# Shashank8834/multimodal-fl-security

Hardware: AMD Instinct MI355X
Metric: FL rounds/sec + aggregate-ms, K=128 clients 10M-param multimodal, 1/2/4/8 GPU (higher is better)
Workload: dtype f32 (bf16x6-split MFMA conv/GEMM = fp32 operands; Krum Gram bf16x4 hi/lo split, fp32 accumulate); 1 GPU; C3: Multi-Krum K=128, 20% sign-flip, ResNet-18 img + 1-layer GRU text late fusion, 5 local SGD steps/round; Krum distances reference-exact; preset=C3, model=resnet18-img+gru1-text late-fusion, clients=128, params=11800394, local_steps=5, batch=32, defense=krum(f=25, multi_k=64), attack=sign_flip, attackers=25, client_chunk=128, exchange=alltoall, krum_distances=reference-exact (fp32 torch.norm accumulation, D bit-identical to krum.py:89-97), training_phase=one captured HIP graph per round; local updates = one flr_train_clients_ex call

## Files before the change

### include/flr.h

```cpp
#ifndef FLR_H
#define FLR_H

#include <stddef.h>
#include <stdint.h>

#ifdef __cplusplus
extern "C" {
#endif

#define FLR_OK 0
#define FLR_ERR_ARG (-1)
#define FLR_ERR_HIP (-2)
#define FLR_ERR_UNSUPPORTED (-3)
#define FLR_ERR_WORKSPACE (-4)
#define FLR_ERR_KRUM_N (-5)

const char* flr_version(void);
const char* flr_build_info(void);
int flr_set_knob(const char* name, const char* value);
const char* flr_status_string(int status);
const char* flr_last_error(void);

size_t flr_pairwise_l2_workspace(int64_t K, int64_t P);
int flr_pairwise_l2(const float* X, int64_t K, int64_t P, int64_t ldx,
// ... 249 lines not shown
                          void* workspace, size_t workspace_bytes, void* stream);
int flr_conv2d_bwd_data_t_add(const float* dy, const float* w_t, const float* add,
                              float* dx, int64_t K, int64_t B, int64_t Cin, int64_t H,
                              int64_t W, int64_t Cout, int64_t KH, int64_t KW,
                              int64_t stride, int64_t pad, void* workspace,
                              size_t workspace_bytes, void* stream);
int flr_conv2d_fwd_t_ex(const float* x, const float* w_t, int64_t w_stride, float* y,
                        int64_t K, int64_t B, int64_t Cin, int64_t H, int64_t W, int64_t Cout,
                        int64_t KH, int64_t KW, int64_t stride, int64_t pad, void* workspace,
                        size_t workspace_bytes, void* stream);
int flr_conv2d_bwd_data_t_ex(const float* dy, const float* w_t, int64_t w_stride,
                             const float* add, float* dx, int64_t K, int64_t B, int64_t Cin,
                             int64_t H, int64_t W, int64_t Cout, int64_t KH, int64_t KW,
                             int64_t stride, int64_t pad, void* workspace,
                             size_t workspace_bytes, void* stream);
int flr_conv2d_resident_ok(int64_t K, int64_t B, int64_t Cin, int64_t H, int64_t W,
                           int64_t Cout, int64_t KH, int64_t KW, int64_t stride,
                           int64_t pad, int dgrad);
int flr_conv2d_bwd_weight_t(const float* x, const float* dy, float* dw_t, int64_t K,
                            int64_t B, int64_t Cin, int64_t H, int64_t W,
                            int64_t Cout, int64_t KH, int64_t KW, int64_t stride,
                            int64_t pad, int zero_dead_taps, void* workspace,
                            size_t workspace_bytes, void* stream);
int64_t flr_conv2d_bwd_weight_t_sq_slots(int64_t K, int64_t B, int64_t Cin, int64_t H,
                                         int64_t W, int64_t Cout, int64_t KH, int64_t KW,
                                         int64_t stride, int64_t pad);
int flr_conv2d_bwd_weight_t_sq(const float* x, const float* dy, float* dw_t, int64_t K,
                               int64_t B, int64_t Cin, int64_t H, int64_t W,
                               int64_t Cout, int64_t KH, int64_t KW, int64_t stride,
                               int64_t pad, int zero_dead_taps, double* sq, int64_t sq_ld,
// ... 190 lines not shown
```

### multimodal-fl-security_amd/csrc/conv_t_kernels.h

```cpp
#pragma once

#include "conv_t_plans.h"

namespace flr {
namespace convt {

__device__ __forceinline__ void xcd_tile(int& bx, int& by, int& bz) {
  const int gx = (int)gridDim.x, gy = (int)gridDim.y;
  const int n = gx * gy * (int)gridDim.z;
  const int lid = (int)blockIdx.x + gx * ((int)blockIdx.y + gy * (int)blockIdx.z);
  const int xcd = lid & 7, slot = lid >> 3;
  const int q = n >> 3, r = n & 7;
  const int t = (xcd < r ? xcd * (q + 1) : r * (q + 1) + (xcd - r) * q) + slot;
  bx = t % gx;
  by = (t / gx) % gy;
  bz = t / (gx * gy);
}

template <class P> struct has_sq : std::false_type {};
template <bool V> struct has_sq<WgtT<V>> : std::true_type {};

__device__ __forceinline__ double block_sumsq(double s, double* red) {
#pragma unroll
  for (int o = 32; o > 0; o >>= 1) s += __shfl_xor(s, o, 64);
// ... 307 lines not shown
  }
}

constexpr int SB = 32;
constexpr int TERM_B = 64 * SB;
__device__ __forceinline__ int zimg(int row, int c) {
  const int f = ((row >> 2) & 1) | ((((row >> 1) ^ (row >> 3)) & 1) << 1);
  return row * SB + 8 * (c ^ f);
}
constexpr int SG_OCC = 2;
template <class P> struct has_k8 : std::false_type {};
template <> struct has_k8<FwdT> : std::true_type {};
template <> struct has_k8<DgradT> : std::true_type {};
template <int A, int B> struct has_k8<BGemm<A, B>> : std::true_type {};
template <class Plan, int MS, int NS, int ABL = 0, bool NAR = false>
__device__ __forceinline__ void sgemm_body(const Plan& pl, int S, float* __restrict__ part, int remap) {
  static_assert(!NAR || (NS == 1 && (MS == 2 || MS == 4)), "narrow tiles: 128 or 256 x 32");
  constexpr int MSW = NAR ? MS / 2 : MS;
  __shared__ __attribute__((aligned(16))) __bf16 Ls[MS + NS][3][TERM_B];
  int bx = (int)blockIdx.x, by = (int)blockIdx.y, bz = (int)blockIdx.z;
  if (remap & 1) xcd_tile(bx, by, bz);
  if (remap >> 8) odd_slot_controls(remap);
  const int k = bz / S, split = bz % S;
  const int M = pl.M(), N = pl.N(), R = pl.R();
  const int ktiles = cdiv(R, BK);
  const int rbeg = (int)((int64_t)ktiles * split / S) * BK;
  const int rend = std::min(R, (int)((int64_t)ktiles * (split + 1) / S) * BK);
  const int m0 = by * BM * MS, n0 = bx * BN * NS;
  const int tid = threadIdx.x;
  const int wave = tid >> 6, lane = tid & 63;
  const int wm = wave >> 1, wn = wave & 1;
  const int h = lane >> 5, l32 = lane & 31;
  const int srowA = stash_row<Plan::QUAD_A>(tid), skA = stash_k<Plan::QUAD_A>(tid);
  const int srowB = stash_row<Plan::QUAD_B>(tid), skB = stash_k<Plan::QUAD_B>(tid);

  typename Plan::State8 sa[MS], sb[NS];
#pragma unroll
  for (int i = 0; i < MS; ++i) sa[i] = pl.init8(k, m0 + BM * i, n0, tid);
#pragma unroll
  for (int j = 0; j < NS; ++j) sb[j] = pl.init8(k, m0, n0 + BN * j, tid);
  float ra[MS][8], rb[NS][8];
  bf16x8 pa[MS][3], pb[NS][3];
  f32x16 acc[MSW][NS];
#pragma unroll
  for (int i = 0; i < MSW; ++i)
#pragma unroll
    for (int j = 0; j < NS; ++j)
#pragma unroll
      for (int e = 0; e < 16; ++e) acc[i][j][e] = 0.f;
  auto a_sub = [&](int i) { return NAR ? (wave * MSW + i) >> 1 : i; };
  auto a_row = [&](int i) { return NAR ? 32 * ((wave * MSW + i) & 1) + l32 : 32 * wm + l32; };
  auto b_row = [&]() { return NAR ? l32 : 32 * wn + l32; };
  auto m_off = [&](int i) { return NAR ? 32 * (wave * MSW + i) : BM * i + 32 * wm; };
  auto n_off = [&](int j) { return NAR ? 0 : BN * j + 32 * wn; };
  auto load = [&](int r) {
#pragma unroll
    for (int i = 0; i < MS; ++i) pl.load_a8(sa[i], r, ra[i]);
#pragma unroll
    for (int j = 0; j < NS; ++j) pl.load_b8(sb[j], r, rb[j]);
  };
  auto split_all = [&]() {
#pragma unroll
    for (int i = 0; i < MS; ++i) split3(ra[i], pa[i][0], pa[i][1], pa[i][2]);
#pragma unroll
    for (int j = 0; j < NS; ++j) split3(rb[j], pb[j][0], pb[j][1], pb[j][2]);
  };
  auto write_all = [&]() {
#pragma unroll
    for (int i = 0; i < MS; ++i)
// ... 38 lines not shown
    split_all();
    write_all();
    load(std::min(rbeg + BK, rlast));
    __syncthreads();
    auto tile_body = [&](int t) {
      const int r0 = rbeg + t * BK;
      if constexpr (!(ABL & 16)) compute_tile();
      if constexpr (!(ABL & 8)) split_all();
      if constexpr (!(ABL & 4)) __syncthreads();
      if constexpr (!(ABL & 2)) write_all();
      if constexpr (!(ABL & 1)) load(std::min(r0 + 2 * BK, rlast));
      __syncthreads();
    };
    for (int t = 0; t < ntile; ++t) tile_body(t);
  }
  TileOffs<MSW, NS> off;
#pragma unroll
  for (int i = 0; i < MSW; ++i) off.m[i] = m_off(i);
#pragma unroll
  for (int j = 0; j < NS; ++j) off.n[j] = n_off(j);
  off.wr = off.wc = 0;
  store_tiles<Plan, MSW, NS>(pl, S, part, k, split, m0, n0, h, l32, M, N, acc, off);
}

template <class Plan, int MS, int NS, int ABL = 0, bool NAR = false>
__global__ __launch_bounds__(THREADS, SG_OCC) void sgemm_kernel(const Plan pl, int S, float* __restrict__ part,
                                                                 int remap) {
  sgemm_body<Plan, MS, NS, ABL, NAR>(pl, S, part, remap);
}

constexpr int RES_N = 128;
constexpr int RES_IMG = (RES_N + 1) * SB;

template <class Plan>
__global__ __launch_bounds__(THREADS, SG_OCC) void rgemm_kernel(const Plan pl, int remap) {
  __shared__ __attribute__((aligned(16))) __bf16 La[3][TERM_B];
  __shared__ __attribute__((aligned(16))) __bf16 Lb[2][3][RES_IMG];
// ... 511 lines not shown
  return v ? v : conv_min_kt();
}

inline int dgrad_min_kt2() {
  static const int v = [] {
    const char* e = flr::knob("FLR_DGRAD_MINKT2");
    const int x = e ? atoi(e) : 0;
    return x >= 1 && x <= 256 ? x : 8;
  }();
  return v;
}

template <class Plan>
inline int plan_min_kt(const Plan& pl) {
  if (std::is_base_of<BGemmArgs, Plan>::value) return bgemm_min_kt();
  if constexpr (std::is_same<Plan, DgradT>::value) return pl.g.stride == 1 ? dgrad_min_kt1() : dgrad_min_kt2();
  return conv_min_kt();
}

template <class Plan>
size_t splits_bytes(const Plan& pl) {
  int S = 1;
  for (int sub : {1, 2, 3, 4}) S = std::max(S, choose_splits(pl.M(), pl.N(), pl.R(), pl.g.Kc, sub, plan_min_kt(pl)));
  return S > 1 ? (size_t)S * pl.g.Kc * pl.M() * pl.N() * sizeof(float) : 0;
}

inline int tile_choice(int M, int N, int R) {
  const char* e = flr::knob("FLR_CONV_TILE");
  const int forced = e ? atoi(e) : 0;
  if (forced == 11) return 11;
  if (forced == 21 && M % 128 == 0) return 21;
// ... 267 lines not shown
      case 13: return launch_tiles<Plan, 1, 3>(pl, ws, ws_bytes, st, name);
      case 31: return launch_tiles<Plan, 3, 1>(pl, ws, ws_bytes, st, name);
      case 14: return launch_tiles<Plan, 1, 4>(pl, ws, ws_bytes, st, name);
      case 41: return launch_tiles<Plan, 4, 1>(pl, ws, ws_bytes, st, name);
      default: break;
    }
  }
  switch (tile) {
    case 21: return launch_tiles<Plan, 2, 1>(pl, ws, ws_bytes, st, name);
    case 12: return launch_tiles<Plan, 1, 2>(pl, ws, ws_bytes, st, name);
    case 22: return launch_tiles<Plan, 2, 2>(pl, ws, ws_bytes, st, name);
    default: return launch_tiles<Plan, 1, 1>(pl, ws, ws_bytes, st, name);
  }
}

inline bool shape_ok(int64_t Cin, int64_t Cout) { return Cin % 64 == 0 && Cout % 64 == 0; }

inline bool args_ok(int64_t K, int64_t B, int64_t Cin, int64_t H, int64_t W, int64_t Cout, int64_t KH, int64_t KW,
                    int64_t stride, int64_t pad) {
  if (!conv::geom_ok(K, B, Cin, H, W, Cout, KH, KW, stride, pad) || !shape_ok(Cin, Cout)) return false;
  if (!(B * K * Cin * H * W * 4 < (int64_t(1) << 31) && B * K * Cout * H * W * 4 < (int64_t(1) << 31) &&
        KH * KW * Cin * Cout * 4 < (int64_t(1) << 31)))
    return false;
  if (stride > 4) return false;
  const conv::Geom g = conv::make_geom(K, B, Cin, H, W, Cout, KH, KW, stride, pad);
  if (!g.rect.ok) return false;
  DgradT cls[MAX_CLASSES];
  const int nc = dgrad_classes(g, cls);
  for (int c = 0; c < nc; ++c)
    if (!cls[c].crect.ok) return false;
// ... 6 lines not shown
```

### multimodal-fl-security_amd/csrc/conv_t_plans.h

```cpp
#pragma once

#include "conv_t_prims.h"

namespace flr {
namespace convt {

struct FwdT {
  static constexpr bool QUAD_A = false, QUAD_B = false;
  Geom g;
  const float* x;
  const float* w;
  float* y;
  int64_t wsk;
  static constexpr int LA = KR_VEC, LB = KR_GATHER;
  __host__ __device__ __forceinline__ int M() const { return g.Cout; }
  __host__ __device__ __forceinline__ int N() const { return g.B * g.Ho * g.Wo; }
  __host__ __device__ __forceinline__ int R() const { return g.ntaps * g.Cin; }
  struct State {
    rsrc_t ra, rb;
    unsigned a0;
    int ih0, iw0, xoff;
    bool nok;
  };
  __device__ __forceinline__ State init(int k, int m0, int n0, int tid) const {
// ... 103 lines not shown
  __device__ __forceinline__ void res_shift(int slot, int& dh, int& dw) const {
    int kh, kw;
    slot_tap(g, slot, kh, kw);
    dh = kh - g.pad;
    dw = kw - g.pad;
  }
};

struct DgradT {
  static constexpr bool QUAD_A = true, QUAD_B = false;
  Geom g;
  const float* dy;
  const float* w;
  float* dx;
  const float* add;
  int64_t wsk;
  int ca, cb, Hc, Wc, ntc;
  conv::FastDiv d_hcwc, d_wc;
  int8_t ckh[conv::MAXTAPS], ckw[conv::MAXTAPS];
  conv::TapRect crect;
  static constexpr int LA = RK_VEC, LB = KR_GATHER;
  __host__ __device__ __forceinline__ int M() const { return g.Cin; }
  __host__ __device__ __forceinline__ int N() const { return g.B * Hc * Wc; }
  __host__ __device__ __forceinline__ int R() const { return ntc * g.Cout; }
  struct State {
    rsrc_t ra, rb;
    unsigned a0;
    int ih, iw, yoff;
    bool nok;
  };
// ... 35 lines not shown
    const int nh = s.ih - kh, nw = s.iw - kw;
    const int oh = g.stride == 1 ? nh : nh / g.stride, ow = g.stride == 1 ? nw : nw / g.stride;
    const bool ok = s.nok & (nh >= 0) & (nw >= 0) & (oh < g.Ho) & (ow < g.Wo);
    const unsigned addr = (unsigned)((s.yoff + oh * g.Wo + ow) * 4);
    const unsigned vb = ok ? addr : SENT;
    const int cs = (int)g.syc;
    const int cb0 = co0 * cs * 4;
#pragma unroll
    for (int i = 0; i < 8; ++i) b[i] = ld1(s.rb, vb, cb0 + i * 4 * cs * 4);
  }
  __device__ __forceinline__ void store(int k, int m, int n, float v) const {
    const uint32_t bb = udiv(n, d_hcwc), p = n - bb * Hc * Wc;
    const uint32_t ihc = udiv(p, d_wc), iwc = p - ihc * Wc;
    const int ih = ca + (int)ihc * g.stride, iw = cb + (int)iwc * g.stride;
    const int64_t i = k * g.sxk + m * g.sxc + bb * g.sxb + ih * g.W + iw;
    dx[i] = add ? __fadd_rn(v, add[i]) : v;
  }
  __device__ __forceinline__ int64_t index(int k, int m, int n) const {
    const uint32_t bb = udiv(n, d_hcwc), p = n - bb * Hc * Wc;
    const uint32_t ihc = udiv(p, d_wc), iwc = p - ihc * Wc;
    const int ih = ca + (int)ihc * g.stride, iw = cb + (int)iwc * g.stride;
    return k * g.sxk + m * g.sxc + bb * g.sxb + ih * g.W + iw;
  }
  __device__ __forceinline__ bool linear() const { return g.stride == 1; }
  __device__ __forceinline__ float* out() const { return dx; }
  __device__ __forceinline__ int64_t tile_base(int k, int m0, int n0) const { return k * g.sxk + m0 * g.sxc + n0; }
  __device__ __forceinline__ int64_t ldm() const { return g.sxc; }
  struct State8 {
    rsrc_t ra, rb;
    unsigned a0;
    int ih, iw, yoff;
    bool nok;
// ... 54 lines not shown
  }
  __device__ __forceinline__ void res_shift(int slot, int& dh, int& dw) const {
    int kh, kw;
    conv::rect_tap(crect, slot, kh, kw);
    dh = g.pad - kh;
    dw = g.pad - kw;
  }
};

inline int dgrad_classes(const Geom& g, DgradT* out) {
  int n = 0;
  for (int ca = 0; ca < std::min(g.stride, g.H); ++ca)
    for (int cb = 0; cb < std::min(g.stride, g.W); ++cb) {
      DgradT& c = out[n++];
      c.g = g;
      c.ca = ca;
      c.cb = cb;
      c.Hc = (g.H - ca + g.stride - 1) / g.stride;
      c.Wc = (g.W - cb + g.stride - 1) / g.stride;
      c.d_hcwc = conv::make_fastdiv((uint32_t)(c.Hc * c.Wc));
      c.d_wc = conv::make_fastdiv((uint32_t)c.Wc);
      c.ntc = 0;
      for (int t = 0; t < g.ntaps; ++t) {
        const int kh = g.tap_kh[t], kw = g.tap_kw[t];
        if (((ca + g.pad - kh) % g.stride + g.stride) % g.stride != 0) continue;
        if (((cb + g.pad - kw) % g.stride + g.stride) % g.stride != 0) continue;
        c.ckh[c.ntc] = (int8_t)kh;
        c.ckw[c.ntc] = (int8_t)kw;
        ++c.ntc;
      }
// ... 661 lines not shown
```

### multimodal-fl-security_amd/csrc/train_clients.hip

```cpp
#include "flr_common.h"
#include "side_stream.h"

#include <algorithm>
#include <cstring>
#include <string>
#include <vector>

namespace flr {
int clip_sumsq_blocks(const float* const* g_blocks, const int64_t* numel, const int64_t* client_stride,
                      int64_t nblocks, int64_t K, double* out, int64_t out_ld, int nslots, hipStream_t st);
namespace tc {

constexpr int THREADS = 256;

__global__ void permute_images_kernel(const float* __restrict__ src, float* __restrict__ dst, int64_t K, int64_t B,
                                      int64_t C, int64_t HW) {
  const int64_t n = K * B * C * HW;
  for (int64_t i = (int64_t)blockIdx.x * THREADS + threadIdx.x; i < n; i += (int64_t)gridDim.x * THREADS) {
    const int64_t p = i % HW, r = i / HW;
    const int64_t b = r % B, r2 = r / B;
    const int64_t c = r2 % C, k = r2 / C;
    dst[i] = src[((k * B + b) * C + c) * HW + p];
  }
}
// ... 415 lines not shown
      t.n[i] = r[i].second;
      total = std::max(total, r[i].second);
    }
    const int64_t g = std::max<int64_t>(1, std::min<int64_t>(256, (total / 4 + THREADS - 1) / THREADS));
    hipLaunchKernelGGL(dead_ranges_kernel, dim3((unsigned)g, (unsigned)K_), dim3(THREADS), 0, st, t, gtrain, X, ld,
                       (int)std::min<int64_t>(nneg, K_));
    return launch_status("train_clients: dead ranges");
  }

  struct Options {
    AuxStream* side = nullptr;
    AuxStream* text = nullptr;
    AuxStream* wgrad = nullptr;
    float* norms = nullptr;
    bool fuse_res = true;
    bool shared_first = true;
    float* xout = nullptr;
    int64_t xld = 0, xneg = 0;
  };
  void configure(const Options& o) { o_ = o; }

  int step(const float* images, const int64_t* tokens, const int64_t* labels, const float* mask, bool first,
           bool last, float* loss_row, float lr, float mom, hipStream_t st) {
    int rc;
    const int64_t C0 = s_.in_channels, HW0 = s_.image_size * s_.image_size;
    const Param& whh = ps_[p_whh_];
    Step S;
    S.st = st;
    S.conc = o_.text != nullptr;
    S.ts = S.conc ? o_.text->s : st;
// ... 218 lines not shown
    return FLR_OK;
  }

  int trunk_backward(Step& S) {
    int rc;
    const hipStream_t st = S.st;
    const int wg_text = S.conc ? [] {
      const char* e = flr::knob("FLR_WG_TEXT");
      return e ? atoi(e) : 2;
    }() : 0;
    for (int bi = (int)blocks_.size() - 1; bi >= 0; --bi) {
      Block& bk = blocks_[bi];
      S.wg_on_text = bi < wg_text;
      const float* d_out = bi + 1 < (int)blocks_.size() ? blocks_[bi + 1].d_in : d_x4_;
      FLR_TRY(bn_bwd(bk.b2, d_out, bk.y2, bk.out, true, bk.d_y2, bk.d_res, st));
      FLR_TRY(conv_bwd(S, bk.c2, bk.a1, bk.d_y2, bk.d_a1, st));
      FLR_TRY(bn_bwd(bk.b1, bk.d_a1, bk.y1, bk.a1, true, bk.d_y1, nullptr, st));
      const float* other = bk.d_res;
      if (bk.has_ds) {
        FLR_TRY(bn_bwd(bk.bds, bk.d_res, bk.yd, nullptr, false, bk.d_yd, nullptr, st));
        if (ps_[bk.c1.p].tap && ps_[bk.ds.p].tap && o_.fuse_res) {
          FLR_TRY(conv_bwd(S, bk.c1, bk.x_in, bk.d_y1, bk.d_in, st));
          FLR_TRY(conv_bwd(S, bk.ds, bk.x_in, bk.d_yd, bk.d_in, st, bk.d_in));
          continue;
        }
        FLR_TRY(conv_bwd(S, bk.ds, bk.x_in, bk.d_yd, bk.d_xd, st));
        other = bk.d_xd;
      }
      if (ps_[bk.c1.p].tap && o_.fuse_res) {
        FLR_TRY(conv_bwd(S, bk.c1, bk.x_in, bk.d_y1, bk.d_in, st, other));
      } else {
        FLR_TRY(conv_bwd(S, bk.c1, bk.x_in, bk.d_y1, bk.d_xm, st));
// ... 171 lines not shown
  const float* tap_w(const Param& p, bool shared, int64_t& stride) const {
    stride = shared ? 0 : p.n;
    return shared ? gshared_ + p.off : p.w;
  }
  int conv_fwd(const Step& S, const ConvOp& c, const float* x, float* y, hipStream_t st, char* wsp = nullptr) {
    const Param& p = ps_[c.p];
    if (p.tap) {
      int64_t wst;
      const float* w = tap_w(p, S.wsh, wst);
      return flr_conv2d_fwd_t_ex(x, w, wst, y, K_, B_, c.Cin, c.H, c.H, c.Cout, c.k, c.k, c.stride, c.pad,
                                 wsp ? wsp : cws_, cws_n_, st);
    }
    return flr_conv2d_fwd(x, p.w, y, K_, B_, c.Cin, c.H, c.H, c.Cout, c.k, c.k, c.stride, c.pad, c.fws, c.fws_n, st);
  }
  int conv_bwd(Step& S, const ConvOp& c, const float* x, const float* dy, float* dx, hipStream_t st,
               const float* add = nullptr) {
    const Param& p = ps_[c.p];
    int rc;
    if (p.tap) {
      int64_t wst;
      const float* w = tap_w(p, S.wsh, wst);
      hipStream_t ws = st;
      char* wsp = cws_;
      if (S.wg_on_text && S.tx.left(2)) {
        FLR_TRY(ev_link(S.tx.take(), st, o_.text->s, "train_clients: text-stream weight-gradient fork"));
        ws = o_.text->s;
        wsp = cws3_;
      } else if (S.wg.left(2)) {
        FLR_TRY(ev_link(S.wg.take(), st, o_.wgrad->s, "train_clients: weight-gradient fork"));
        ws = o_.wgrad->s;
        wsp = cws2_;
      }
      if (dx && (rc = flr_conv2d_bwd_data_t_ex(dy, w, wst, add, dx, K_, B_, c.Cin, c.H, c.H, c.Cout, c.k, c.k,
                                               c.stride, c.pad, cws_, cws_n_, st)) != FLR_OK)
        return rc;
      const int zero_dead = p.dead ? 0 : 1;
      if (p.sq_base >= 0)
        return flr_conv2d_bwd_weight_t_sq(x, dy, p.g, K_, B_, c.Cin, c.H, c.H, c.Cout, c.k, c.k, c.stride, c.pad,
                                          zero_dead, sq_ + p.sq_base, std::max<int64_t>(1, nsq_), wsp, cws_n_, ws);
      return flr_conv2d_bwd_weight_t(x, dy, p.g, K_, B_, c.Cin, c.H, c.H, c.Cout, c.k, c.k, c.stride, c.pad, zero_dead,
                                     wsp, cws_n_, ws);
    }
    if (dx && (rc = flr_conv2d_bwd_data(dy, p.w, dx, K_, B_, c.Cin, c.H, c.H, c.Cout, c.k, c.k, c.stride, c.pad, cws_,
                                        cws_n_, st)) != FLR_OK)
      return rc;
    return flr_conv2d_bwd_weight_reuse(x, dy, p.g, K_, B_, c.Cin, c.H, c.H, c.Cout, c.k, c.k, c.stride, c.pad, c.fws,
                                       c.fws_n, st);
  }
  int bn_fwd(const BnOp& b, const float* x, const float* res, float* y, bool relu, hipStream_t st) {
    return flr_batchnorm_fwd(x, ps_[b.pg].w, ps_[b.pb].w, res, y, b.mean, b.invstd, 1, K_ * b.C, b.HW, 1e-5f,
                             relu ? 1 : 0, st);
  }
  int bn_bwd(const BnOp& b, const float* dy, const float* x, const float* y, bool relu, float* dx, float* dres,
             hipStream_t st) {
    return flr_batchnorm_bwd(dy, x, relu ? y : nullptr, ps_[b.pg].w, b.mean, b.invstd, dx, ps_[b.pg].g, ps_[b.pb].g,
                             dres, 1, K_ * b.C, b.HW, relu ? 1 : 0, st);
  }
  int gemm(const float* A, int64_t ak, int64_t am, int64_t ar, const float* Bm, int64_t bk, int64_t bn, int64_t br,
           float* C, int64_t ck, int64_t cm, int64_t cn, const float* bias, int64_t bias_k, const float* add,
           int64_t M, int64_t N, int64_t R, hipStream_t st) {
    return flr_bgemm(A, ak, am, ar, Bm, bk, bn, br, C, ck, cm, cn, bias, bias_k, add, K_, M, N, R, gws_, gws_n_, st);
  }
// ... 89 lines not shown
  float* step_loss = reinterpret_cast<float*>(base + align_up(net.bytes(), 256));
  static const bool fuse_res = [] {
    const char* e = flr::knob("FLR_FUSED_RES");
    return !(e && e[0] == '0');
  }();
  static const bool shared_first = [] {
    const char* e = flr::knob("FLR_SHARED_FIRST");
    return !(e && e[0] == '0');
  }();
  const bool train_order = (flags & FLR_TC_TRAIN_ORDER) != 0;
  hipStream_t st = as_stream(stream);
  tc::Net::Options o;
  o.norms = norms_out;
  o.fuse_res = fuse_res;
  o.shared_first = shared_first;
  o.side = side_stream(true, st);
  o.text = text_stream(true, st);
  o.wgrad = wgrad_stream(true, st);
  if (train_order) {
    o.xout = X;
    o.xld = ld;
    o.xneg = nneg;
  }
  net.configure(o);
  rc = train_order ? net.load_global_train(global, st) : net.load_global(global, st);
  if (rc != FLR_OK) return rc;
  const int64_t C0 = spec->in_channels, HW0 = spec->image_size * spec->image_size, T = spec->seq_len;
  for (int64_t s = 0; s < steps; ++s) {
    rc = net.step(images + s * K * B * C0 * HW0, tokens + s * K * B * T, labels + s * K * B,
                  dropout_masks ? dropout_masks + s * K * B * spec->fusion : nullptr, s == 0, s == steps - 1,
// ... 51 lines not shown
```

### multimodal-fl-security_amd/csrc/train_conv_t_dgrad.hip

```cpp
#include "conv_t_kernels.h"

using namespace flr;

extern "C" int flr_conv2d_bwd_data_t(const float* dy, const float* w_t, float* dx, int64_t K, int64_t B, int64_t Cin,
                                     int64_t H, int64_t W, int64_t Cout, int64_t KH, int64_t KW, int64_t stride,
                                     int64_t pad, void* ws, size_t ws_bytes, void* stream) {
  return flr_conv2d_bwd_data_t_add(dy, w_t, nullptr, dx, K, B, Cin, H, W, Cout, KH, KW, stride, pad, ws, ws_bytes,
                                   stream);
}

extern "C" int flr_conv2d_bwd_data_t_add(const float* dy, const float* w_t, const float* add, float* dx, int64_t K,
                                         int64_t B, int64_t Cin, int64_t H, int64_t W, int64_t Cout, int64_t KH,
                                         int64_t KW, int64_t stride, int64_t pad, void* ws, size_t ws_bytes,
                                         void* stream) {
  return flr_conv2d_bwd_data_t_ex(dy, w_t, KH * KW * Cin * Cout, add, dx, K, B, Cin, H, W, Cout, KH, KW, stride, pad,
                                  ws, ws_bytes, stream);
}

extern "C" int flr_conv2d_bwd_data_t_ex(const float* dy, const float* w_t, int64_t w_stride, const float* add,
                                        float* dx, int64_t K, int64_t B, int64_t Cin, int64_t H, int64_t W,
                                        int64_t Cout, int64_t KH, int64_t KW, int64_t stride, int64_t pad, void* ws,
                                        size_t ws_bytes, void* stream) {
  if (!dy || !w_t || !dx || w_stride < 0) return FLR_ERR_ARG;
  if (!convt::args_ok(K, B, Cin, H, W, Cout, KH, KW, stride, pad))
    return conv::geom_ok(K, B, Cin, H, W, Cout, KH, KW, stride, pad) ? FLR_ERR_UNSUPPORTED : FLR_ERR_ARG;
  if (stride > 4) return FLR_ERR_UNSUPPORTED;
  const conv::Geom g = conv::make_geom(K, B, Cin, H, W, Cout, KH, KW, stride, pad);
  convt::DgradT cls[convt::MAX_CLASSES];
  const int nc = convt::dgrad_classes(g, cls);
  for (int c = 0; c < nc; ++c) {
    if (add == dx && cls[c].R() == 0) continue;
    cls[c].dy = dy; cls[c].w = w_t; cls[c].dx = dx; cls[c].add = add; cls[c].wsk = w_stride;
    const int rc = convt::launch(cls[c], ws, ws_bytes, as_stream(stream), "conv bwd data (tap-major)");
    if (rc != FLR_OK) return rc;
  }
  return FLR_OK;
}
```

### multimodal-fl-security_amd/flr/_capi.py

```python
from __future__ import annotations

import ctypes
import os
import threading

import torch

_PKG_ROOT = os.path.dirname(os.path.dirname(os.path.abspath(__file__)))
LIB_PATH = os.environ.get("FLR_LIB", os.path.join(_PKG_ROOT, "lib", "libflr.so"))
HEADER_PATH = os.path.join(os.path.dirname(_PKG_ROOT), "include", "flr.h")

FLR_OK = 0
FLR_ERR_ARG = -1
FLR_ERR_HIP = -2
FLR_ERR_UNSUPPORTED = -3
FLR_ERR_WORKSPACE = -4
FLR_ERR_KRUM_N = -5

_c_void_p = ctypes.c_void_p
_i64 = ctypes.c_int64
_size_t = ctypes.c_size_t
_int = ctypes.c_int

SIGNATURES = {
# ... 116 lines not shown
    "flr_vit_bert_num_params": (_i64, [_c_void_p]),
    "flr_train_vit_bert_workspace": (_size_t, [_c_void_p, _i64, _i64, _i64, _i64]),
    "flr_train_vit_bert": (_int, [_c_void_p, _c_void_p, _c_void_p, _i64, _c_void_p, _c_void_p, _c_void_p,
                                  _c_void_p, _i64, _i64, _i64, ctypes.c_float, ctypes.c_float, ctypes.c_float,
                                  ctypes.c_float, _i64, _c_void_p, _c_void_p, ctypes.c_uint, _i64, _c_void_p,
                                  _size_t, _c_void_p]),
    "flr_conv2d_tap_major_ok": (_int, [_i64, _i64]),
    "flr_conv2d_t_workspace": (_size_t, [_i64] * 10),
    "flr_conv2d_fwd_t": (_int, [_c_void_p, _c_void_p, _c_void_p] + [_i64] * 10 + [_c_void_p, _size_t, _c_void_p]),
    "flr_conv2d_bwd_data_t": (_int, [_c_void_p, _c_void_p, _c_void_p] + [_i64] * 10 + [_c_void_p, _size_t, _c_void_p]),
    "flr_conv2d_bwd_data_t_add": (_int, [_c_void_p] * 4 + [_i64] * 10 + [_c_void_p, _size_t, _c_void_p]),
    "flr_conv2d_fwd_t_ex": (_int, [_c_void_p, _c_void_p, _i64, _c_void_p] + [_i64] * 10 + [_c_void_p, _size_t,
                                                                                          _c_void_p]),
    "flr_conv2d_bwd_data_t_ex": (_int, [_c_void_p, _c_void_p, _i64, _c_void_p, _c_void_p] + [_i64] * 10 +
                                 [_c_void_p, _size_t, _c_void_p]),
    "flr_conv2d_resident_ok": (_int, [_i64] * 10 + [_int]),
    "flr_conv2d_bwd_weight_t": (_int, [_c_void_p, _c_void_p, _c_void_p] + [_i64] * 10 + [_int, _c_void_p, _size_t,
                                                                                         _c_void_p]),
    "flr_conv2d_bwd_weight_t_sq_slots": (_i64, [_i64] * 10),
    "flr_conv2d_wgrad_resident_ok": (_int, [_i64] * 10),
    "flr_conv2d_bwd_weight_t_sq": (_int, [_c_void_p, _c_void_p, _c_void_p] + [_i64] * 10 + [_int, _c_void_p, _i64,
                                                                                            _c_void_p, _size_t,
                                                                                            _c_void_p]),
    "flr_conv2d_fwd": (_int, [_c_void_p, _c_void_p, _c_void_p] + [_i64] * 10 + [_c_void_p, _size_t, _c_void_p]),
    "flr_conv2d_bwd_data": (_int, [_c_void_p, _c_void_p, _c_void_p] + [_i64] * 10 + [_c_void_p, _size_t, _c_void_p]),
    "flr_conv2d_bwd_weight": (_int, [_c_void_p, _c_void_p, _c_void_p] + [_i64] * 10 + [_c_void_p, _size_t, _c_void_p]),
    "flr_conv2d_bwd_weight_reuse": (_int, [_c_void_p, _c_void_p, _c_void_p] + [_i64] * 10 + [_c_void_p, _size_t,
                                                                                            _c_void_p]),
    "flr_cross_entropy": (_int, [_c_void_p, _c_void_p, _i64, _i64, _i64, _c_void_p, _c_void_p, _c_void_p, _c_void_p]),
    "flr_mean_rows": (_int, [_c_void_p, _i64, _i64, _c_void_p, _c_void_p]),
# ... 132 lines not shown
```

Before: 17.65 rounds/s.

## Merge strided dgrad phase classes into one launch and fold shortcut gradient early

Adds a merged dgrad kernel that handles all stride-phase classes of a strided convolution in a single launch, doing split-K reduction in registers instead of through workspace partials. It also computes the 1x1 stride-2 downsample shortcut gradient into a compact buffer early, optionally on the wgrad side stream, and folds it into the main conv1 dgrad epilogue in place of a separate add pass. This removes several small launches and partial-sum traffic in ResNet backward. The cost is less parallelism per tile, since splits are serialized inside a block, plus extra stream fork/join events.

```diff
diff --git a/include/flr.h b/include/flr.h
--- a/include/flr.h
+++ b/include/flr.h
@@ -287,6 +287,15 @@
                              int64_t H, int64_t W, int64_t Cout, int64_t KH, int64_t KW,
                              int64_t stride, int64_t pad, void* workspace,
                              size_t workspace_bytes, void* stream);
+int flr_conv2d_bwd_data_t_ex2(const float* dy, const float* w_t, int64_t w_stride,
+                              const float* add, const float* add_c, float* dx,
+                              int compact_out, int64_t K, int64_t B, int64_t Cin, int64_t H,
+                              int64_t W, int64_t Cout, int64_t KH, int64_t KW, int64_t stride,
+                              int64_t pad, void* workspace, size_t workspace_bytes,
+                              void* stream);
+int flr_conv2d_dgrad_merged_ok(int64_t K, int64_t B, int64_t Cin, int64_t H, int64_t W,
+                               int64_t Cout, int64_t KH, int64_t KW, int64_t stride,
+                               int64_t pad);
 int flr_conv2d_resident_ok(int64_t K, int64_t B, int64_t Cin, int64_t H, int64_t W,
                            int64_t Cout, int64_t KH, int64_t KW, int64_t stride,
                            int64_t pad, int dgrad);
diff --git a/multimodal-fl-security_amd/csrc/conv_t_kernels.h b/multimodal-fl-security_amd/csrc/conv_t_kernels.h
--- a/multimodal-fl-security_amd/csrc/conv_t_kernels.h
+++ b/multimodal-fl-security_amd/csrc/conv_t_kernels.h
@@ -345,19 +345,11 @@
 template <> struct has_k8<DgradT> : std::true_type {};
 template <int A, int B> struct has_k8<BGemm<A, B>> : std::true_type {};
 template <class Plan, int MS, int NS, int ABL = 0, bool NAR = false>
-__device__ __forceinline__ void sgemm_body(const Plan& pl, int S, float* __restrict__ part, int remap) {
+__device__ __forceinline__ void sgemm_acc(const Plan& pl, int k, int m0, int n0, int rbeg, int rend,
+                                          f32x16 (&acc)[NAR ? MS / 2 : MS][NS]) {
   static_assert(!NAR || (NS == 1 && (MS == 2 || MS == 4)), "narrow tiles: 128 or 256 x 32");
   constexpr int MSW = NAR ? MS / 2 : MS;
   __shared__ __attribute__((aligned(16))) __bf16 Ls[MS + NS][3][TERM_B];
-  int bx = (int)blockIdx.x, by = (int)blockIdx.y, bz = (int)blockIdx.z;
-  if (remap & 1) xcd_tile(bx, by, bz);
-  if (remap >> 8) odd_slot_controls(remap);
-  const int k = bz / S, split = bz % S;
-  const int M = pl.M(), N = pl.N(), R = pl.R();
-  const int ktiles = cdiv(R, BK);
-  const int rbeg = (int)((int64_t)ktiles * split / S) * BK;
-  const int rend = std::min(R, (int)((int64_t)ktiles * (split + 1) / S) * BK);
-  const int m0 = by * BM * MS, n0 = bx * BN * NS;
   const int tid = threadIdx.x;
   const int wave = tid >> 6, lane = tid & 63;
   const int wm = wave >> 1, wn = wave & 1;
@@ -372,7 +364,6 @@
   for (int j = 0; j < NS; ++j) sb[j] = pl.init8(k, m0, n0 + BN * j, tid);
   float ra[MS][8], rb[NS][8];
   bf16x8 pa[MS][3], pb[NS][3];
-  f32x16 acc[MSW][NS];
 #pragma unroll
   for (int i = 0; i < MSW; ++i)
 #pragma unroll
@@ -382,8 +373,6 @@
   auto a_sub = [&](int i) { return NAR ? (wave * MSW + i) >> 1 : i; };
   auto a_row = [&](int i) { return NAR ? 32 * ((wave * MSW + i) & 1) + l32 : 32 * wm + l32; };
   auto b_row = [&]() { return NAR ? l32 : 32 * wn + l32; };
-  auto m_off = [&](int i) { return NAR ? 32 * (wave * MSW + i) : BM * i + 32 * wm; };
-  auto n_off = [&](int j) { return NAR ? 0 : BN * j + 32 * wn; };
   auto load = [&](int r) {
 #pragma unroll
     for (int i = 0; i < MS; ++i) pl.load_a8(sa[i], r, ra[i]);
@@ -452,13 +441,81 @@
     };
     for (int t = 0; t < ntile; ++t) tile_body(t);
   }
+}
+template <int MS, int NS, bool NAR>
+__device__ __forceinline__ TileOffs<(NAR ? MS / 2 : MS), NS> sgemm_offs() {
+  constexpr int MSW = NAR ? MS / 2 : MS;
+  const int wave = (int)threadIdx.x >> 6, wm = wave >> 1, wn = wave & 1;
   TileOffs<MSW, NS> off;
 #pragma unroll
-  for (int i = 0; i < MSW; ++i) off.m[i] = m_off(i);
-#pragma unroll
-  for (int j = 0; j < NS; ++j) off.n[j] = n_off(j);
+  for (int i = 0; i < MSW; ++i) off.m[i] = NAR ? 32 * (wave * MSW + i) : BM * i + 32 * wm;
+#pragma unroll
+  for (int j = 0; j < NS; ++j) off.n[j] = NAR ? 0 : BN * j + 32 * wn;
   off.wr = off.wc = 0;
-  store_tiles<Plan, MSW, NS>(pl, S, part, k, split, m0, n0, h, l32, M, N, acc, off);
+  return off;
+}
+
+template <class Plan, int MS, int NS, int ABL = 0, bool NAR = false>
+__device__ __forceinline__ void sgemm_body(const Plan& pl, int S, float* __restrict__ part, int remap) {
+  constexpr int MSW = NAR ? MS / 2 : MS;
+  int bx = (int)blockIdx.x, by = (int)blockIdx.y, bz = (int)blockIdx.z;
+  if (remap & 1) xcd_tile(bx, by, bz);
+  if (remap >> 8) odd_slot_controls(remap);
+  const int k = bz / S, split = bz % S;
+  const int M = pl.M(), N = pl.N(), R = pl.R();
+  const int ktiles = cdiv(R, BK);
+  const int rbeg = (int)((int64_t)ktiles * split / S) * BK;
+  const int rend = std::min(R, (int)((int64_t)ktiles * (split + 1) / S) * BK);
+  const int m0 = by * BM * MS, n0 = bx * BN * NS;
+  const int lane = (int)threadIdx.x & 63;
+  f32x16 acc[MSW][NS];
+  sgemm_acc<Plan, MS, NS, ABL, NAR>(pl, k, m0, n0, rbeg, rend, acc);
+  store_tiles<Plan, MSW, NS>(pl, S, part, k, split, m0, n0, lane >> 5, lane & 31, M, N, acc, sgemm_offs<MS, NS, NAR>());
+}
+
+constexpr int MG_CLASSES = 4;
+struct DgradSet {
+  DgradT c[MG_CLASSES];
+  int S[MG_CLASSES];
+  int tn[MG_CLASSES];
+  int t0[MG_CLASSES + 1];
+  int nc;
+};
+template <int MS, int NS, bool NAR>
+__global__ __launch_bounds__(THREADS, SG_OCC) void mgemm_kernel(const DgradSet set, int remap) {
+  constexpr int MSW = NAR ? MS / 2 : MS;
+  int bx = (int)blockIdx.x, by = (int)blockIdx.y, bz = (int)blockIdx.z;
+  if (remap & 1) xcd_tile(bx, by, bz);
+  int ci = 0;
+#pragma unroll
+  for (int i = 1; i < MG_CLASSES; ++i)
+    if (i < set.nc && bx >= set.t0[i]) ci = i;
+  ci = uni(ci);
+  const DgradT& pl = set.c[ci];
+  const int S = set.S[ci], t = bx - set.t0[ci];
+  const int tm = t / set.tn[ci], tnn = t - tm * set.tn[ci];
+  const int k = bz;
+  const int M = pl.M(), N = pl.N(), R = pl.R();
+  const int ktiles = cdiv(R, BK);
+  const int m0 = tm * BM * MS, n0 = tnn * BN * NS;
+  const int lane = (int)threadIdx.x & 63;
+  f32x16 acc[MSW][NS], prt[MSW][NS];
+  for (int split = 0; split < S; ++split) {
+    const int rbeg = (int)((int64_t)ktiles * split / S) * BK;
+    const int rend = std::min(R, (int)((int64_t)ktiles * (split + 1) / S) * BK);
+    if (split == 0) {
+      sgemm_acc<DgradT, MS, NS, 0, NAR>(pl, k, m0, n0, rbeg, rend, acc);
+    } else {
+      sgemm_acc<DgradT, MS, NS, 0, NAR>(pl, k, m0, n0, rbeg, rend, prt);
+#pragma unroll
+      for (int i = 0; i < MSW; ++i)
+#pragma unroll
+        for (int j = 0; j < NS; ++j)
+#pragma unroll
+          for (int e = 0; e < 16; ++e) acc[i][j][e] += prt[i][j][e];
+    }
+  }
+  store_tiles<DgradT, MSW, NS>(pl, 1, nullptr, k, 0, m0, n0, lane >> 5, lane & 31, M, N, acc, sgemm_offs<MS, NS, NAR>());
 }
 
 template <class Plan, int MS, int NS, int ABL = 0, bool NAR = false>
@@ -1000,7 +1057,8 @@
 template <class Plan>
 inline int plan_min_kt(const Plan& pl) {
   if (std::is_base_of<BGemmArgs, Plan>::value) return bgemm_min_kt();
-  if constexpr (std::is_same<Plan, DgradT>::value) return pl.g.stride == 1 ? dgrad_min_kt1() : dgrad_min_kt2();
+  if constexpr (std::is_same<Plan, DgradT>::value)
+    return pl.min_kt ? pl.min_kt : (pl.g.stride == 1 ? dgrad_min_kt1() : dgrad_min_kt2());
   return conv_min_kt();
 }
 
@@ -1298,6 +1356,60 @@
   }
 }
 
+inline int dgrad_merged() {
+  const char* e = flr::knob("FLR_DGRAD_MERGED");
+  return e ? atoi(e) : 1;
+}
+inline int plan_merged(const DgradT* cls, int nc, const void* ws, size_t ws_bytes, DgradSet& set, bool& nar_form) {
+  const int mode = dgrad_merged();
+  if (mode == 0 || nc < 2 || nc > MG_CLASSES || gemm_form() != 5) return 0;
+  const int K = cls[0].g.Kc, M = cls[0].M();
+  int narrow = 0, wide = 0;
+  set.nc = nc;
+  int order[MG_CLASSES];
+  for (int i = 0; i < nc; ++i) order[i] = i;
+  std::stable_sort(order, order + nc, [&](int a, int b) { return cls[a].R() > cls[b].R(); });
+  for (int i = 0; i < nc; ++i) {
+    const DgradT& c = cls[order[i]];
+    if (c.R() == 0) return 0;
+    const bool nar = c.N() <= 32 && c.M() % (2 * BM) == 0 && conv_narrow();
+    narrow += nar;
+    wide += c.N() % (2 * BN) == 0;
+    const int tile = plan_tile(c);
+    int S = choose_splits(c.M(), c.N(), c.R(), K, nar ? 2 : (tile / 10) * (tile % 10), plan_min_kt(c));
+    if (S > 1 && (!ws || ws_bytes < (size_t)S * K * c.M() * c.N() * sizeof(float))) S = 1;
+    set.c[i] = c;
+    set.S[i] = S;
+  }
+  if (narrow != 0 && narrow != nc) return 0;
+  const int ms = narrow ? 2 : 1, ns = (!narrow && M == BM && wide == nc) ? 2 : 1;
+  int t = 0;
+  for (int i = 0; i < nc; ++i) {
+    set.tn[i] = cdiv(set.c[i].N(), BN * ns);
+    set.t0[i] = t;
+    t += set.tn[i] * cdiv(M, BM * ms);
+  }
+  set.t0[nc] = t;
+  for (int i = nc; i < MG_CLASSES; ++i) set.S[i] = set.tn[i] = 1;
+  if (mode != 2 && (int64_t)t * K < FILL_WG) return 0;
+  nar_form = narrow != 0;
+  return 10 * ms + ns;
+}
+inline int launch_merged(const DgradT* cls, int nc, const void* ws, size_t ws_bytes, hipStream_t st, const char* name) {
+  DgradSet set;
+  bool narrow = false;
+  const int tile = plan_merged(cls, nc, ws, ws_bytes, set, narrow);
+  if (tile == 0) return FLR_ERR_UNSUPPORTED;
+  const dim3 grid((unsigned)set.t0[nc], 1u, (unsigned)cls[0].g.Kc);
+  if (narrow)
+    hipLaunchKernelGGL((mgemm_kernel<2, 1, true>), grid, dim3(THREADS), 0, st, set, xcd_remap() & 1);
+  else if (tile % 10 == 2)
+    hipLaunchKernelGGL((mgemm_kernel<1, 2, false>), grid, dim3(THREADS), 0, st, set, xcd_remap() & 1);
+  else
+    hipLaunchKernelGGL((mgemm_kernel<1, 1, false>), grid, dim3(THREADS), 0, st, set, xcd_remap() & 1);
+  return launch_status(name);
+}
+
 inline bool shape_ok(int64_t Cin, int64_t Cout) { return Cin % 64 == 0 && Cout % 64 == 0; }
 
 inline bool args_ok(int64_t K, int64_t B, int64_t Cin, int64_t H, int64_t W, int64_t Cout, int64_t KH, int64_t KW,
diff --git a/multimodal-fl-security_amd/csrc/conv_t_plans.h b/multimodal-fl-security_amd/csrc/conv_t_plans.h
--- a/multimodal-fl-security_amd/csrc/conv_t_plans.h
+++ b/multimodal-fl-security_amd/csrc/conv_t_plans.h
@@ -141,6 +141,8 @@
   const float* w;
   float* dx;
   const float* add;
+  const float* addc;
+  int min_kt;
   int64_t wsk;
   int ca, cb, Hc, Wc, ntc;
   conv::FastDiv d_hcwc, d_wc;
@@ -206,8 +208,10 @@
     const uint32_t ihc = udiv(p, d_wc), iwc = p - ihc * Wc;
     const int ih = ca + (int)ihc * g.stride, iw = cb + (int)iwc * g.stride;
     const int64_t i = k * g.sxk + m * g.sxc + bb * g.sxb + ih * g.W + iw;
+    if (addc) v = __fadd_rn(addc[compact(k, m, n)], v);
     dx[i] = add ? __fadd_rn(v, add[i]) : v;
   }
+  __device__ __forceinline__ int64_t compact(int k, int m, int n) const { return ((int64_t)k * M() + m) * N() + n; }
   __device__ __forceinline__ int64_t index(int k, int m, int n) const {
     const uint32_t bb = udiv(n, d_hcwc), p = n - bb * Hc * Wc;
     const uint32_t ihc = udiv(p, d_wc), iwc = p - ihc * Wc;
@@ -292,6 +296,8 @@
     for (int cb = 0; cb < std::min(g.stride, g.W); ++cb) {
       DgradT& c = out[n++];
       c.g = g;
+      c.add = c.addc = nullptr;
+      c.min_kt = 0;
       c.ca = ca;
       c.cb = cb;
       c.Hc = (g.H - ca + g.stride - 1) / g.stride;
diff --git a/multimodal-fl-security_amd/csrc/train_clients.hip b/multimodal-fl-security_amd/csrc/train_clients.hip
--- a/multimodal-fl-security_amd/csrc/train_clients.hip
+++ b/multimodal-fl-security_amd/csrc/train_clients.hip
@@ -453,6 +453,7 @@
     AuxStream* wgrad = nullptr;
     float* norms = nullptr;
     bool fuse_res = true;
+    bool ds_early = true;
     bool shared_first = true;
     float* xout = nullptr;
     int64_t xld = 0, xneg = 0;
@@ -701,8 +702,36 @@
       S.wg_on_text = bi < wg_text;
       const float* d_out = bi + 1 < (int)blocks_.size() ? blocks_[bi + 1].d_in : d_x4_;
       FLR_TRY(bn_bwd(bk.b2, d_out, bk.y2, bk.out, true, bk.d_y2, bk.d_res, st));
+      const bool ds_early = bk.has_ds && o_.ds_early && o_.fuse_res && ps_[bk.c1.p].tap && ps_[bk.ds.p].tap &&
+                            bk.ds.k == 1 && bk.ds.pad == 0 && bk.ds.stride >= 2 && bk.ds.stride == bk.c1.stride &&
+                            bk.ds.H == bk.c1.H && bk.ds.Cin == bk.c1.Cin;
+      hipEvent_t ds_done = nullptr;
+      if (ds_early) {
+        const bool side = S.wg.left(3);
+        const hipStream_t dst = side ? o_.wgrad->s : st;
+        char* wsp = side ? cws2_ : cws_;
+        if (side) FLR_TRY(ev_link(S.wg.take(), st, dst, "train_clients: shortcut gradient fork"));
+        FLR_TRY(bn_bwd(bk.bds, bk.d_res, bk.yd, nullptr, false, bk.d_yd, nullptr, dst));
+        {
+          const ConvOp& c = bk.ds;
+          int64_t wst;
+          const float* w = tap_w(ps_[c.p], S.wsh, wst);
+          FLR_TRY(flr_conv2d_bwd_data_t_ex2(bk.d_yd, w, wst, nullptr, nullptr, bk.d_xd, 1, K_, B_, c.Cin, c.H, c.H,
+                                            c.Cout, c.k, c.k, c.stride, c.pad, wsp, cws_n_, dst));
+        }
+        if (side) {
+          ds_done = S.wg.take();
+          FLR_TRY(ev_record(ds_done, dst, "train_clients: shortcut gradient event"));
+        }
+        FLR_TRY(conv_wgrad(bk.ds, bk.x_in, bk.d_yd, wsp, dst));
+      }
       FLR_TRY(conv_bwd(S, bk.c2, bk.a1, bk.d_y2, bk.d_a1, st));
       FLR_TRY(bn_bwd(bk.b1, bk.d_a1, bk.y1, bk.a1, true, bk.d_y1, nullptr, st));
+      if (ds_early) {
+        if (ds_done) FLR_TRY(ev_wait(st, ds_done, "train_clients: shortcut gradient join"));
+        FLR_TRY(conv_bwd(S, bk.c1, bk.x_in, bk.d_y1, bk.d_in, st, nullptr, bk.d_xd));
+        continue;
+      }
       const float* other = bk.d_res;
       if (bk.has_ds) {
         FLR_TRY(bn_bwd(bk.bds, bk.d_res, bk.yd, nullptr, false, bk.d_yd, nullptr, st));
@@ -904,7 +933,7 @@
     return flr_conv2d_fwd(x, p.w, y, K_, B_, c.Cin, c.H, c.H, c.Cout, c.k, c.k, c.stride, c.pad, c.fws, c.fws_n, st);
   }
   int conv_bwd(Step& S, const ConvOp& c, const float* x, const float* dy, float* dx, hipStream_t st,
-               const float* add = nullptr) {
+               const float* add = nullptr, const float* add_c = nullptr) {
     const Param& p = ps_[c.p];
     int rc;
     if (p.tap) {
@@ -921,21 +950,25 @@
         ws = o_.wgrad->s;
         wsp = cws2_;
       }
-      if (dx && (rc = flr_conv2d_bwd_data_t_ex(dy, w, wst, add, dx, K_, B_, c.Cin, c.H, c.H, c.Cout, c.k, c.k,
-                                               c.stride, c.pad, cws_, cws_n_, st)) != FLR_OK)
+      if (dx && (rc = flr_conv2d_bwd_data_t_ex2(dy, w, wst, add, add_c, dx, 0, K_, B_, c.Cin, c.H, c.H, c.Cout, c.k,
+                                                c.k, c.stride, c.pad, cws_, cws_n_, st)) != FLR_OK)
         return rc;
-      const int zero_dead = p.dead ? 0 : 1;
-      if (p.sq_base >= 0)
-        return flr_conv2d_bwd_weight_t_sq(x, dy, p.g, K_, B_, c.Cin, c.H, c.H, c.Cout, c.k, c.k, c.stride, c.pad,
-                                          zero_dead, sq_ + p.sq_base, std::max<int64_t>(1, nsq_), wsp, cws_n_, ws);
-      return flr_conv2d_bwd_weight_t(x, dy, p.g, K_, B_, c.Cin, c.H, c.H, c.Cout, c.k, c.k, c.stride, c.pad, zero_dead,
-                                     wsp, cws_n_, ws);
+      return conv_wgrad(c, x, dy, wsp, ws);
     }
     if (dx && (rc = flr_conv2d_bwd_data(dy, p.w, dx, K_, B_, c.Cin, c.H, c.H, c.Cout, c.k, c.k, c.stride, c.pad, cws_,
                                         cws_n_, st)) != FLR_OK)
       return rc;
     return flr_conv2d_bwd_weight_reuse(x, dy, p.g, K_, B_, c.Cin, c.H, c.H, c.Cout, c.k, c.k, c.stride, c.pad, c.fws,
                                        c.fws_n, st);
+  }
+  int conv_wgrad(const ConvOp& c, const float* x, const float* dy, char* wsp, hipStream_t ws) {
+    const Param& p = ps_[c.p];
+    const int zero_dead = p.dead ? 0 : 1;
+    if (p.sq_base >= 0)
+      return flr_conv2d_bwd_weight_t_sq(x, dy, p.g, K_, B_, c.Cin, c.H, c.H, c.Cout, c.k, c.k, c.stride, c.pad,
+                                        zero_dead, sq_ + p.sq_base, std::max<int64_t>(1, nsq_), wsp, cws_n_, ws);
+    return flr_conv2d_bwd_weight_t(x, dy, p.g, K_, B_, c.Cin, c.H, c.H, c.Cout, c.k, c.k, c.stride, c.pad, zero_dead,
+                                   wsp, cws_n_, ws);
   }
   int bn_fwd(const BnOp& b, const float* x, const float* res, float* y, bool relu, hipStream_t st) {
     return flr_batchnorm_fwd(x, ps_[b.pg].w, ps_[b.pb].w, res, y, b.mean, b.invstd, 1, K_ * b.C, b.HW, 1e-5f,
@@ -1055,6 +1088,10 @@
   o.norms = norms_out;
   o.fuse_res = fuse_res;
   o.shared_first = shared_first;
+  {
+    const char* e = flr::knob("FLR_DGRAD_MERGED");
+    o.ds_early = !(e && e[0] == '0');
+  }
   o.side = side_stream(true, st);
   o.text = text_stream(true, st);
   o.wgrad = wgrad_stream(true, st);
diff --git a/multimodal-fl-security_amd/csrc/train_conv_t_dgrad.hip b/multimodal-fl-security_amd/csrc/train_conv_t_dgrad.hip
--- a/multimodal-fl-security_amd/csrc/train_conv_t_dgrad.hip
+++ b/multimodal-fl-security_amd/csrc/train_conv_t_dgrad.hip
@@ -21,16 +21,57 @@
                                         float* dx, int64_t K, int64_t B, int64_t Cin, int64_t H, int64_t W,
                                         int64_t Cout, int64_t KH, int64_t KW, int64_t stride, int64_t pad, void* ws,
                                         size_t ws_bytes, void* stream) {
+  return flr_conv2d_bwd_data_t_ex2(dy, w_t, w_stride, add, nullptr, dx, 0, K, B, Cin, H, W, Cout, KH, KW, stride, pad,
+                                   ws, ws_bytes, stream);
+}
+
+extern "C" int flr_conv2d_dgrad_merged_ok(int64_t K, int64_t B, int64_t Cin, int64_t H, int64_t W, int64_t Cout,
+                                          int64_t KH, int64_t KW, int64_t stride, int64_t pad) {
+  if (stride < 2 || stride > 4 || !convt::args_ok(K, B, Cin, H, W, Cout, KH, KW, stride, pad)) return 0;
+  const conv::Geom g = conv::make_geom(K, B, Cin, H, W, Cout, KH, KW, stride, pad);
+  convt::DgradT cls[convt::MAX_CLASSES];
+  const int nc = convt::dgrad_classes(g, cls);
+  convt::DgradSet set;
+  bool narrow = false;
+  return convt::plan_merged(cls, nc, &set, SIZE_MAX, set, narrow) != 0 ? 1 : 0;
+}
+
+extern "C" int flr_conv2d_bwd_data_t_ex2(const float* dy, const float* w_t, int64_t w_stride, const float* add,
+                                         const float* add_c, float* dx, int compact_out, int64_t K, int64_t B,
+                                         int64_t Cin, int64_t H, int64_t W, int64_t Cout, int64_t KH, int64_t KW,
+                                         int64_t stride, int64_t pad, void* ws, size_t ws_bytes, void* stream) {
   if (!dy || !w_t || !dx || w_stride < 0) return FLR_ERR_ARG;
+  if ((add_c || compact_out) && (add || stride < 2)) return FLR_ERR_ARG;
+  if (add_c && compact_out) return FLR_ERR_ARG;
   if (!convt::args_ok(K, B, Cin, H, W, Cout, KH, KW, stride, pad))
     return conv::geom_ok(K, B, Cin, H, W, Cout, KH, KW, stride, pad) ? FLR_ERR_UNSUPPORTED : FLR_ERR_ARG;
   if (stride > 4) return FLR_ERR_UNSUPPORTED;
   const conv::Geom g = conv::make_geom(K, B, Cin, H, W, Cout, KH, KW, stride, pad);
   convt::DgradT cls[convt::MAX_CLASSES];
   const int nc = convt::dgrad_classes(g, cls);
+  if (compact_out) {
+    if (KH != 1 || KW != 1 || pad != 0) return FLR_ERR_UNSUPPORTED;
+    const convt::DgradT& c0 = cls[0];
+    if (!convt::args_ok(K, B, Cin, c0.Hc, c0.Wc, Cout, 1, 1, 1, 0)) return FLR_ERR_UNSUPPORTED;
+    const conv::Geom gc = conv::make_geom(K, B, Cin, c0.Hc, c0.Wc, Cout, 1, 1, 1, 0);
+    if (gc.Ho != g.Ho || gc.Wo != g.Wo) return FLR_ERR_UNSUPPORTED;
+    convt::DgradT one[convt::MAX_CLASSES];
+    if (convt::dgrad_classes(gc, one) != 1 || one[0].M() != c0.M() || one[0].N() != c0.N() || one[0].R() != c0.R())
+      return FLR_ERR_UNSUPPORTED;
+    one[0].dy = dy; one[0].w = w_t; one[0].dx = dx; one[0].wsk = w_stride;
+    one[0].min_kt = convt::dgrad_min_kt2();
+    return convt::launch(one[0], ws, ws_bytes, as_stream(stream), "conv bwd data (tap-major, compact)");
+  }
+  for (int c = 0; c < nc; ++c) {
+    cls[c].dy = dy; cls[c].w = w_t; cls[c].dx = dx; cls[c].add = add; cls[c].wsk = w_stride;
+    cls[c].addc = c == 0 ? add_c : nullptr;
+  }
+  if (stride > 1) {
+    const int rc = convt::launch_merged(cls, nc, ws, ws_bytes, as_stream(stream), "conv bwd data (tap-major, merged)");
+    if (rc != FLR_ERR_UNSUPPORTED) return rc;
+  }
   for (int c = 0; c < nc; ++c) {
     if (add == dx && cls[c].R() == 0) continue;
-    cls[c].dy = dy; cls[c].w = w_t; cls[c].dx = dx; cls[c].add = add; cls[c].wsk = w_stride;
     const int rc = convt::launch(cls[c], ws, ws_bytes, as_stream(stream), "conv bwd data (tap-major)");
     if (rc != FLR_OK) return rc;
   }
diff --git a/multimodal-fl-security_amd/flr/_capi.py b/multimodal-fl-security_amd/flr/_capi.py
--- a/multimodal-fl-security_amd/flr/_capi.py
+++ b/multimodal-fl-security_amd/flr/_capi.py
@@ -154,6 +154,9 @@
                                                                                           _c_void_p]),
     "flr_conv2d_bwd_data_t_ex": (_int, [_c_void_p, _c_void_p, _i64, _c_void_p, _c_void_p] + [_i64] * 10 +
                                  [_c_void_p, _size_t, _c_void_p]),
+    "flr_conv2d_bwd_data_t_ex2": (_int, [_c_void_p, _c_void_p, _i64, _c_void_p, _c_void_p, _c_void_p, _int] +
+                                  [_i64] * 10 + [_c_void_p, _size_t, _c_void_p]),
+    "flr_conv2d_dgrad_merged_ok": (_int, [_i64] * 10),
     "flr_conv2d_resident_ok": (_int, [_i64] * 10 + [_int]),
     "flr_conv2d_bwd_weight_t": (_int, [_c_void_p, _c_void_p, _c_void_p] + [_i64] * 10 + [_int, _c_void_p, _size_t,
                                                                                          _c_void_p]),
```

Result: no change. 17.64 rounds/s, median of 2 (-0.1%).
